# spcl/gemm_hls

Measured on AMD Instinct MI355X. Metric: GFLOP/s, fp32 GEMM N=K=M=16384 per MI355X (tiled outer-product C=A.B), and % of fp32 MFMA peak, higher is better.
Workload: dtype f32; 1 GPU; float 16384x16384x16384 (Multiply,Add) on 1 MI355X; BASELINE configs[1]; kernel=mfma_f32_256x256x16_w8_flush4096, rows_total=16384, rows_per_gpu=16384

## Files before the change

### gemm_hls_amd/csrc/mm_mfma_f32_split.hip

```cpp
#include <mutex>
#include <type_traits>

#include "mm_common.h"

namespace mm {
namespace {

using bf16x8 = __attribute__((ext_vector_type(8))) __bf16;
using f32x4 = __attribute__((ext_vector_type(4))) float;
using f32x16 = __attribute__((ext_vector_type(16))) float;

struct Packed {
  static constexpr int FRAG_BYTES = 64 * 16;
  static constexpr int PLANE_BYTES = 8 * FRAG_BYTES;
  static constexpr int SLAB_BYTES = 3 * PLANE_BYTES;
};
template <int FR_, int WM_, int WN_, int TM_>
struct GeoT {
  static constexpr int FR = FR_, BM = 32 * FR_, BN = 32 * FR_, WM = WM_, WN = WN_, THREADS = 64 * WM_ * WN_;
  static constexpr int TM = TM_, TN = 2, NS = 3;
  static_assert(WM * TM == FR && WN * TN == FR && WM * WN == FR, "one wavefront per fragment and per DMA piece");
  static constexpr int FRAG_BYTES = Packed::FRAG_BYTES;
  static constexpr int PLANE_BYTES = FR * FRAG_BYTES;
  static constexpr int SLAB_BYTES = 3 * PLANE_BYTES;
  static constexpr int STAGE_BYTES = 2 * SLAB_BYTES;
  static constexpr int LDS_BYTES = NS * STAGE_BYTES;
  static constexpr int HALVES = 8 / FR;
};
using GeoS = GeoT<8, 2, 4, 4>;
using GeoS128 = GeoT<4, 2, 2, 2>;

__device__ __forceinline__ void split3(float x, __bf16 &p1, __bf16 &p2, __bf16 &p3) {
  p1 = (__bf16)x;
  const float r1 = x - (float)p1;
  p2 = (__bf16)r1;
  const float r2 = r1 - (float)p2;
  p3 = (__bf16)r2;
  if (!(__builtin_fabsf((float)p1) < __builtin_inff())) {
    p2 = (__bf16)0.0f;
    p3 = (__bf16)0.0f;
  }
}

template <bool ALONG_K, bool PAIRED>
__global__ __launch_bounds__(512) void split_pack_kernel(const float *__restrict__ src, char *__restrict__ dst,
                                                         unsigned rows, unsigned K, unsigned ld, unsigned slabs) {
  const unsigned slab = blockIdx.x, blk = blockIdx.y;
  const unsigned frag = threadIdx.x >> 6, lane = threadIdx.x & 63u;
  const unsigned r = blk * 256 + (PAIRED ? (frag >> 1) * 64 + 2 * (lane & 31u) + (frag & 1u) : frag * 32 + (lane & 31u));
  const unsigned k0 = slab * 16 + (lane >> 5) * 8;
  float x[8];
  if (ALONG_K) {
    if (r < rows && k0 + 8 <= K && (ld & 3u) == 0) {
      const f32x4 lo = *(const f32x4 *)(src + (size_t)r * ld + k0), hi = *(const f32x4 *)(src + (size_t)r * ld + k0 + 4);
#pragma unroll
      for (int e = 0; e < 4; ++e) { x[e] = lo[e]; x[4 + e] = hi[e]; }
    } else {
#pragma unroll
      for (int e = 0; e < 8; ++e) x[e] = (r < rows && k0 + e < K) ? src[(size_t)r * ld + k0 + e] : 0.0f;
    }
  } else {
#pragma unroll
    for (int e = 0; e < 8; ++e) x[e] = (r < rows && k0 + e < K) ? src[(size_t)(k0 + e) * ld + r] : 0.0f;
  }
  bf16x8 p1, p2, p3;
#pragma unroll
  for (int e = 0; e < 8; ++e) {
    __bf16 a, b, c;
    split3(x[e], a, b, c);
    p1[e] = a; p2[e] = b; p3[e] = c;
  }
  char *out = dst + ((size_t)blk * slabs + slab) * Packed::SLAB_BYTES + frag * Packed::FRAG_BYTES + lane * 16;
  *(bf16x8 *)(out) = p1;
  *(bf16x8 *)(out + Packed::PLANE_BYTES) = p2;
  *(bf16x8 *)(out + 2 * Packed::PLANE_BYTES) = p3;
}

__device__ __forceinline__ const char *uniform(const char *p) {
  const unsigned long long v = (unsigned long long)p;
  const unsigned lo = __builtin_amdgcn_readfirstlane((unsigned)v), hi = __builtin_amdgcn_readfirstlane((unsigned)(v >> 32));
  return (const char *)(((unsigned long long)hi << 32) | lo);
}

template <int VAR, int TERMS, class G = GeoS>
__global__ __launch_bounds__(G::THREADS, 2)
void mfma_f32_split_kernel(const char *__restrict__ Ap, const char *__restrict__ Bp, float *__restrict__ C, unsigned N,
                           unsigned M, unsigned slabs, unsigned tiles_n, unsigned tiles_m, unsigned kBand) {
  constexpr int TM = G::TM, TN = G::TN;
  constexpr int NP = TERMS == 6 ? 3 : 2;
  extern __shared__ __attribute__((aligned(16))) char smem[];
  const unsigned lane = threadIdx.x & 63u;
  const unsigned wave = __builtin_amdgcn_readfirstlane(threadIdx.x >> 6);
  constexpr bool PP = (VAR & 64) != 0;
  static_assert(!PP || G::THREADS == 512, "the ping-pong schedule pairs wavefronts w and w+4 of one workgroup");
  const unsigned group = wave >> 2;
  const unsigned wm = PP ? (wave & 3u) >> 1 : wave / G::WN;
  const unsigned wn = PP ? (wave & 1u) * 2 + group : wave % G::WN;
  const unsigned lo = lane & 31u, hi = lane >> 5;

  const unsigned lin = xcd_remap(blockIdx.x, tiles_n * tiles_m);
  const unsigned band = lin / (kBand * tiles_m), within = lin % (kBand * tiles_m);
  const unsigned rows_in_band = min(kBand, tiles_n - band * kBand);
  const unsigned tile_r = band * kBand + within % rows_in_band, tile_c = within / rows_in_band;

  const unsigned voff0 = wave * 1024 + lane * 16, voff1 = voff0 + 8 * 1024, voff2 = voff0 + 16 * 1024;
  const char *a_base = Ap + (size_t)(tile_r / G::HALVES) * slabs * Packed::SLAB_BYTES + (tile_r % G::HALVES) * G::FR * Packed::FRAG_BYTES;
  const char *b_base = Bp + (size_t)(tile_c / G::HALVES) * slabs * Packed::SLAB_BYTES + (tile_c % G::HALVES) * G::FR * Packed::FRAG_BYTES;
  const unsigned lds0 = (unsigned)(size_t)(__attribute__((address_space(3))) char *)smem;
  auto issue = [&](unsigned slab, unsigned buf) {
    const unsigned sl = min(slab, slabs - 1);
    const char *ap = uniform(a_base + (size_t)sl * Packed::SLAB_BYTES), *bp = uniform(b_base + (size_t)sl * Packed::SLAB_BYTES);
    const unsigned la = lds0 + buf * G::STAGE_BYTES + wave * 1024, lb = la + G::SLAB_BYTES;
    unsigned keep;
#define MM_PIECE(vo, sb, la) "s_mov_b32 m0, " la "\n\ts_nop 0\n\tglobal_load_lds_dwordx4 " vo ", " sb "\n\t"
    if constexpr (NP == 3) {
      const unsigned la1 = la + G::PLANE_BYTES, la2 = la + 2 * G::PLANE_BYTES, lb1 = lb + G::PLANE_BYTES, lb2 = lb + 2 * G::PLANE_BYTES;
      asm volatile("s_mov_b32 %0, m0\n\t" MM_PIECE("%1", "%4", "%6") MM_PIECE("%2", "%4", "%7") MM_PIECE("%3", "%4", "%8")
                       MM_PIECE("%1", "%5", "%9") MM_PIECE("%2", "%5", "%10") MM_PIECE("%3", "%5", "%11") "s_mov_b32 m0, %0"
                   : "=&s"(keep)
                   : "v"(voff0), "v"(voff1), "v"(voff2), "s"(ap), "s"(bp), "s"(la), "s"(la1), "s"(la2), "s"(lb), "s"(lb1),
                     "s"(lb2)
                   : "memory");
    } else {
      const unsigned la1 = la + G::PLANE_BYTES, lb1 = lb + G::PLANE_BYTES;
      asm volatile("s_mov_b32 %0, m0\n\t" MM_PIECE("%1", "%3", "%5") MM_PIECE("%2", "%3", "%6") MM_PIECE("%1", "%4", "%7")
                       MM_PIECE("%2", "%4", "%8") "s_mov_b32 m0, %0"
                   : "=&s"(keep)
                   : "v"(voff0), "v"(voff1), "s"(ap), "s"(bp), "s"(la), "s"(la1), "s"(lb), "s"(lb1)
                   : "memory");
    }
#undef MM_PIECE
  };
  constexpr int PIECES = 2 * NP;

  const unsigned a_off = (wm * TM) * G::FRAG_BYTES + lane * 16;
  const unsigned b_off = G::SLAB_BYTES + (wn * TN) * G::FRAG_BYTES + lane * 16;

  f32x16 acc[TM][TN];
#pragma unroll
  for (int mi = 0; mi < TM; ++mi)
#pragma unroll
    for (int ni = 0; ni < TN; ++ni) acc[mi][ni] = (f32x16)0.0f;

  bf16x8 af[2][3], bf[2][TN][3];
  auto read_a = [&](const char *stage, int mi, bf16x8 (&dst)[3]) {
#pragma unroll
    for (int p = 0; p < NP; ++p) dst[p] = *(const bf16x8 *)(stage + a_off + mi * G::FRAG_BYTES + p * G::PLANE_BYTES);
  };
  auto read_b = [&](const char *stage, bf16x8 (&dst)[TN][3]) {
#pragma unroll
    for (int ni = 0; ni < TN; ++ni)
#pragma unroll
      for (int p = 0; p < NP; ++p) dst[ni][p] = *(const bf16x8 *)(stage + b_off + ni * G::FRAG_BYTES + p * G::PLANE_BYTES);
  };
  auto mac = [&](int mi, const bf16x8 (&a)[3], const bf16x8 (&b)[TN][3]) {
    constexpr int PA6[6] = {0, 2, 1, 0, 1, 0}, PB6[6] = {2, 0, 1, 1, 0, 0};
    constexpr int PA3[3] = {0, 1, 0}, PB3[3] = {1, 0, 0};
    if ((VAR & 1) && !(VAR & 16)) __builtin_amdgcn_s_setprio(1);
#pragma unroll
    for (int t = 0; t < TERMS; ++t)
#pragma unroll
      for (int ni = 0; ni < TN; ++ni) {
        const int pa = TERMS == 6 ? PA6[t] : PA3[t % 3], pb = TERMS == 6 ? PB6[t] : PB3[t % 3];
        acc[mi][ni] = __builtin_amdgcn_mfma_f32_32x32x16_bf16(a[pa], b[ni][pb], acc[mi][ni], 0, 0, 0);
      }
    if ((VAR & 1) && !(VAR & 16)) __builtin_amdgcn_s_setprio(0);
  };
  auto sync = [&]() {
    __builtin_amdgcn_sched_barrier(0);
    __builtin_amdgcn_s_barrier();
    __builtin_amdgcn_sched_barrier(0);
  };

  auto stage = [&](auto bufc, auto parc, unsigned s) {
    constexpr int BUF = decltype(bufc)::value, PAR = decltype(parc)::value;
    const char *cur = smem + BUF * G::STAGE_BYTES, *nxt = smem + ((BUF + 1) % 3) * G::STAGE_BYTES;
#pragma unroll
    for (int mi = 0; mi + 1 < TM; ++mi) {
      read_a(cur, mi + 1, af[(mi + 1) & 1]);
      mac(mi, af[mi & 1], bf[PAR]);
    }
    if constexpr (VAR & 16) {
#pragma unroll
      for (int grp = 0; grp + 1 < TM; ++grp) {
#pragma unroll
        for (int i = 0; i < NP; ++i) {
          __builtin_amdgcn_sched_group_barrier(0x008, 1, 0);
          __builtin_amdgcn_sched_group_barrier(0x100, 1, 0);
        }
        __builtin_amdgcn_sched_group_barrier(0x008, 2 * TERMS - NP, 0);
      }
    }
    if constexpr (PIECES == 6) asm volatile("s_waitcnt vmcnt(6)\n\ts_waitcnt lgkmcnt(0)" ::: "memory");
    else asm volatile("s_waitcnt vmcnt(4)\n\ts_waitcnt lgkmcnt(0)" ::: "memory");
    sync();
    issue(s + 3, BUF);
    read_b(nxt, bf[PAR ^ 1]);
    read_a(nxt, 0, af[0]);
    mac(TM - 1, af[(TM - 1) & 1], bf[PAR]);
    if constexpr (VAR & 16) {
      constexpr int READS = (TN + 1) * NP, MFMAS = 2 * TERMS;
#pragma unroll
      for (int i = 0; i < (READS < MFMAS ? READS : MFMAS); ++i) {
        __builtin_amdgcn_sched_group_barrier(0x008, 1, 0);
        __builtin_amdgcn_sched_group_barrier(0x100, 1, 0);
      }
      if (MFMAS > READS) __builtin_amdgcn_sched_group_barrier(0x008, MFMAS - READS, 0);
      else if (READS > MFMAS) __builtin_amdgcn_sched_group_barrier(0x100, READS - MFMAS, 0);
    }
  };

  bf16x8 paf[TM][3];
  auto pp_stage = [&](auto bufc, unsigned s) {
    constexpr int BUF = decltype(bufc)::value;
    const char *cur = smem + BUF * G::STAGE_BYTES;
    read_b(cur, bf[0]);
#pragma unroll
    for (int mi = 0; mi < TM; ++mi) read_a(cur, mi, paf[mi]);
    issue(s + 2, (BUF + 2) % 3);
    if constexpr (PIECES == 6) asm volatile("s_waitcnt vmcnt(6)\n\ts_waitcnt lgkmcnt(0)" ::: "memory");
    else asm volatile("s_waitcnt vmcnt(4)\n\ts_waitcnt lgkmcnt(0)" ::: "memory");
    sync();
    __builtin_amdgcn_s_setprio(1);
#pragma unroll
    for (int mi = 0; mi < TM; ++mi) mac(mi, paf[mi], bf[0]);
    __builtin_amdgcn_s_setprio(0);
    sync();
  };

  const bool shifted = PP && group == 1;
  issue(0, 0);
  issue(1, 1);
  if constexpr (PP) {
    if constexpr (PIECES == 6) asm volatile("s_waitcnt vmcnt(6)" ::: "memory");
    else asm volatile("s_waitcnt vmcnt(4)" ::: "memory");
    sync();
    if (shifted) sync();
  } else {
    issue(2, 2);
    if constexpr (PIECES == 6) asm volatile("s_waitcnt vmcnt(12)" ::: "memory");
    else asm volatile("s_waitcnt vmcnt(8)" ::: "memory");
    sync();
    read_b(smem, bf[0]);
    read_a(smem, 0, af[0]);
  }
  using I0 = std::integral_constant<int, 0>;
  using I1 = std::integral_constant<int, 1>;
  using I2 = std::integral_constant<int, 2>;

  const unsigned row_w = tile_r * G::BM + wm * (TM * 32), col_w = tile_c * G::BN + wn * 64, col = col_w + 2 * lo;
  char *const c_wave = (char *)uniform((const char *)(C + (size_t)row_w * M + col_w));
  const bool pairs = (M & 1u) == 0 && ((size_t)C & 7u) == 0;
  auto writeback = [&](bool accumulate, auto finalc) {
    constexpr bool FINAL = decltype(finalc)::value;
    constexpr int BATCH = FINAL ? 16 : 8;
    using f32x2 = __attribute__((ext_vector_type(2))) float;
    unsigned Mv = M;
    asm volatile("" : "+s"(Mv));
    const unsigned lane_off = (4 * hi * Mv + 2 * lo) * 4u;
    const unsigned rows_left = N > row_w ? N - row_w : 0u;
    const bool interior = pairs && row_w + TM * 32 <= N && col_w + 64 <= M;
    if (interior) {
      typedef __attribute__((address_space(1))) f32x2 *gpair_t;
#pragma unroll
      for (int mi = 0; mi < TM; ++mi)
#pragma unroll
        for (int half = 0; half < 16 / BATCH; ++half) {
          f32x2 old[BATCH];
          if (accumulate) {
#pragma unroll
            for (int j = 0; j < BATCH; ++j) {
              const int rr = half * BATCH + j, lrow = mi * 32 + (rr & 3) + 8 * (rr >> 2);
              old[j] = *(gpair_t)(c_wave + (lane_off + (unsigned)lrow * Mv * 4u));
            }
          } else {
#pragma unroll
            for (int j = 0; j < BATCH; ++j) old[j] = f32x2{0.0f, 0.0f};
          }
#pragma unroll
          for (int j = 0; j < BATCH; ++j) {
            const int rr = half * BATCH + j, lrow = mi * 32 + (rr & 3) + 8 * (rr >> 2);
            *(gpair_t)(c_wave + (lane_off + (unsigned)lrow * Mv * 4u)) = f32x2{acc[mi][0][rr], acc[mi][1][rr]} + old[j];
          }
          if (!FINAL) __builtin_amdgcn_sched_barrier(0);
        }
      return;
    }
#pragma unroll
    for (int mi = 0; mi < TM; ++mi)
#pragma unroll
      for (int half = 0; half < 16 / BATCH; ++half) {
        f32x2 old[BATCH];
#pragma unroll
        for (int j = 0; j < BATCH; ++j) {
          const int rr = half * BATCH + j, lrow = mi * 32 + (rr & 3) + 8 * (rr >> 2);
          const float *src = (const float *)(c_wave + (lane_off + (unsigned)lrow * Mv * 4u));
          const bool row_ok = lrow + 4 * hi < rows_left;
          old[j] = f32x2{0.0f, 0.0f};
          if (accumulate && row_ok) {
            if (pairs) { if (col < M) old[j] = *(const f32x2 *)src; }
            else {
              if (col < M) old[j][0] = src[0];
              if (col + 1 < M) old[j][1] = src[1];
            }
          }
        }
#pragma unroll
        for (int j = 0; j < BATCH; ++j) {
          const int rr = half * BATCH + j, lrow = mi * 32 + (rr & 3) + 8 * (rr >> 2);
          float *dst = (float *)(c_wave + (lane_off + (unsigned)lrow * Mv * 4u));
          const bool row_ok = lrow + 4 * hi < rows_left;
          const f32x2 v = f32x2{acc[mi][0][rr], acc[mi][1][rr]} + old[j];
          if (row_ok) {
            if (pairs) { if (col < M) *(f32x2 *)dst = v; }
            else {
              if (col < M) dst[0] = v[0];
              if (col + 1 < M) dst[1] = v[1];
            }
          }
        }
        if (!FINAL) __builtin_amdgcn_sched_barrier(0);
      }
  };

  constexpr unsigned FC = (VAR & 2) ? ~0u / 2 / 6 * 6 : ((VAR & 32) ? 258 : 516);
  bool flushed = false;
  unsigned c0 = 0, cend = min(FC, slabs);
  for (;;) {
    for (unsigned s = c0; s < cend; s += 6) {
      if constexpr (PP) {
        pp_stage(I0{}, s);
        if (s + 1 < cend) pp_stage(I1{}, s + 1);
        if (s + 2 < cend) pp_stage(I2{}, s + 2);
        if (s + 3 < cend) pp_stage(I0{}, s + 3);
        if (s + 4 < cend) pp_stage(I1{}, s + 4);
        if (s + 5 < cend) pp_stage(I2{}, s + 5);
        continue;
      }
      stage(I0{}, I0{}, s);
      if (s + 1 < cend) stage(I1{}, I1{}, s + 1);
      if (s + 2 < cend) stage(I2{}, I0{}, s + 2);
      if (s + 3 < cend) stage(I0{}, I1{}, s + 3);
      if (s + 4 < cend) stage(I1{}, I0{}, s + 4);
      if (s + 5 < cend) stage(I2{}, I1{}, s + 5);
    }
    if (cend >= slabs) break;
    asm volatile("s_waitcnt vmcnt(0)" ::: "memory");
    writeback(flushed, std::false_type{});
#pragma unroll
    for (int mi = 0; mi < TM; ++mi)
#pragma unroll
      for (int ni = 0; ni < TN; ++ni) acc[mi][ni] = (f32x16)0.0f;
    asm volatile("s_waitcnt vmcnt(0)" ::: "memory");
    flushed = true;
    c0 = cend;
    cend = min(cend + FC, slabs);
  }
  asm volatile("s_waitcnt vmcnt(0)" ::: "memory");
  if (PP && !shifted) sync();
  writeback(flushed, std::true_type{});
}

template <int VAR, int TERMS, class G = GeoS>
int launch_gemm(hipStream_t s, const char *ap, const char *bp, const Problem &p, unsigned slabs) {
  static unsigned long long configured = 0;
  const unsigned tiles_n = (p.n + G::BM - 1) / G::BM, tiles_m = (p.m + G::BN - 1) / G::BN;
  if (int e = ensure_dynamic_lds((const void *)mfma_f32_split_kernel<VAR, TERMS, G>, G::LDS_BYTES, configured)) return e;
  hipLaunchKernelGGL((mfma_f32_split_kernel<VAR, TERMS, G>), dim3(tiles_n * tiles_m), dim3(G::THREADS), G::LDS_BYTES, s, ap,
                     bp, (float *)p.c, p.n, p.m, slabs, tiles_n, tiles_m, band_rows());
  return (int)hipGetLastError();
}

}

bool mfma_f32_split_serves(const Problem &p) { return p.n > 0 && p.m > 0 && p.k > 0 && 132ull * p.m * 4ull < (1ull << 32); }

int mfma_f32_split_tile(const Problem &p, int variant) {
  if (variant > 0 && (variant & 256)) return 256;
  if (variant > 0 && (variant & 512)) return 128;
  static const TileCandidate cands[] = {{256, 256, 256, 1, 1.0}, {128, 128, 128, 2, 0.85}};
  return pick_tile(cands, 2, p.n, p.m);
}

size_t mfma_f32_split_workspace_bytes(const Problem &p) {
  const size_t slabs = (p.k + 15) / 16;
  return ((size_t)((p.n + 255) / 256) + (size_t)((p.m + 255) / 256)) * slabs * Packed::SLAB_BYTES;
}


int launch_mfma_f32_split(hipStream_t s, const Problem &p, int variant) {
  const unsigned slabs = (p.k + 15) / 16;
  const unsigned blocks_a = (p.n + 255) / 256, blocks_b = (p.m + 255) / 256;
  const size_t a_bytes = (size_t)blocks_a * slabs * Packed::SLAB_BYTES, b_bytes = (size_t)blocks_b * slabs * Packed::SLAB_BYTES;
  int dev = 0;
  hipError_t e = hipGetDevice(&dev);
  if (e != hipSuccess) return (int)e;
  hipMemPool_t pool = nullptr;
  if (int rc = workspace_pool(dev, &pool)) return rc;
  char *ws = nullptr;
  const int v = variant < 0 ? 0 : variant;
  if (v & 48) return kErrNotSupported;
  const bool sync_alloc = v & 8;
  if (sync_alloc) e = hipMalloc((void **)&ws, a_bytes + b_bytes);
  else e = hipMallocFromPoolAsync((void **)&ws, a_bytes + b_bytes, pool, s);
  if (e != hipSuccess) return (int)e;
  const float *a = (const float *)p.a, *b = (const float *)p.b;
  (void)hipGetLastError();
  if (p.a_transposed)
    hipLaunchKernelGGL((split_pack_kernel<false, false>), dim3(slabs, blocks_a), dim3(512), 0, s, a, ws, p.n, p.k, p.n, slabs);
  else
    hipLaunchKernelGGL((split_pack_kernel<true, false>), dim3(slabs, blocks_a), dim3(512), 0, s, a, ws, p.n, p.k, p.k, slabs);
  int rc = (int)hipGetLastError();
  if (rc == 0) {
    hipLaunchKernelGGL((split_pack_kernel<false, true>), dim3(slabs, blocks_b), dim3(512), 0, s, b, ws + a_bytes, p.m, p.k, p.m,
                       slabs);
    rc = (int)hipGetLastError();
  }
  if (rc == 0) {
    const char *bp = ws + a_bytes;
    if (v & 1) rc = launch_gemm<1, 6>(s, ws, bp, p, slabs);
    else if ((v & 128) && (v & 4)) rc = launch_gemm<16 | 2, 6>(s, ws, bp, p, slabs);
    else if (v & 128) rc = launch_gemm<16, 6>(s, ws, bp, p, slabs);
    else if (v & 2) rc = launch_gemm<64, 3>(s, ws, bp, p, slabs);
    else if (v & 4) rc = launch_gemm<64 | 2, 6>(s, ws, bp, p, slabs);
    else if (v & 64) rc = launch_gemm<64 | 32, 6>(s, ws, bp, p, slabs);
    else if (mfma_f32_split_tile(p, v) == 128) rc = launch_gemm<16, 6, GeoS128>(s, ws, bp, p, slabs);
    else rc = launch_gemm<64, 6>(s, ws, bp, p, slabs);
  }
  hipError_t f;
  if (sync_alloc) { f = hipStreamSynchronize(s); (void)hipFree(ws); }
  else f = hipFreeAsync(ws, s);
  return rc ? rc : (int)f;
}

}
```

Measured before the change: 150,500 GFLOP/s.

## Switch split-bf16 GEMM body to 16x16x32 MFMA with paired split products

```diff
diff --git a/gemm_hls_amd/csrc/mm_mfma_f32_split.hip b/gemm_hls_amd/csrc/mm_mfma_f32_split.hip
--- a/gemm_hls_amd/csrc/mm_mfma_f32_split.hip
+++ b/gemm_hls_amd/csrc/mm_mfma_f32_split.hip
@@ -42,13 +42,17 @@
   }
 }
 
-template <bool ALONG_K, bool PAIRED>
+template <bool ALONG_K, bool PAIRED, bool H16>
 __global__ __launch_bounds__(512) void split_pack_kernel(const float *__restrict__ src, char *__restrict__ dst,
                                                          unsigned rows, unsigned K, unsigned ld, unsigned slabs) {
   const unsigned slab = blockIdx.x, blk = blockIdx.y;
   const unsigned frag = threadIdx.x >> 6, lane = threadIdx.x & 63u;
-  const unsigned r = blk * 256 + (PAIRED ? (frag >> 1) * 64 + 2 * (lane & 31u) + (frag & 1u) : frag * 32 + (lane & 31u));
-  const unsigned k0 = slab * 16 + (lane >> 5) * 8;
+  const unsigned slot = H16 ? (lane & 15u) + 16 * (lane >> 5) : lane & 31u, kgroup = H16 ? (lane >> 4) & 1u : lane >> 5;
+  const unsigned in_block = !PAIRED ? frag * 32 + slot
+                            : H16   ? frag * 32 + 2 * (slot & 15u) + (slot >> 4)
+                                    : (frag >> 1) * 64 + 2 * slot + (frag & 1u);
+  const unsigned r = blk * 256 + in_block;
+  const unsigned k0 = slab * 16 + kgroup * 8;
   float x[8];
   if (ALONG_K) {
     if (r < rows && k0 + 8 <= K && (ld & 3u) == 0) {
@@ -87,6 +91,8 @@
 void mfma_f32_split_kernel(const char *__restrict__ Ap, const char *__restrict__ Bp, float *__restrict__ C, unsigned N,
                            unsigned M, unsigned slabs, unsigned tiles_n, unsigned tiles_m, unsigned kBand) {
   constexpr int TM = G::TM, TN = G::TN;
+  constexpr bool I32 = (VAR & 128) != 0, SWAP = (VAR & 256) != 0, ADDR = !I32 && !SWAP;
+  static_assert(I32 ? !SWAP : TERMS == 6, "the 16x16x32 body pairs the six products; three products stay on 32x32x16");
   constexpr int NP = TERMS == 6 ? 3 : 2;
   extern __shared__ __attribute__((aligned(16))) char smem[];
   const unsigned lane = threadIdx.x & 63u;
@@ -133,37 +139,86 @@
   };
   constexpr int PIECES = 2 * NP;
 
-  const unsigned a_off = (wm * TM) * G::FRAG_BYTES + lane * 16;
-  const unsigned b_off = G::SLAB_BYTES + (wn * TN) * G::FRAG_BYTES + lane * 16;
-
-  f32x16 acc[TM][TN];
-#pragma unroll
-  for (int mi = 0; mi < TM; ++mi)
-#pragma unroll
-    for (int ni = 0; ni < TN; ++ni) acc[mi][ni] = (f32x16)0.0f;
-
-  bf16x8 af[2][3], bf[2][TN][3];
-  auto read_a = [&](const char *stage, int mi, bf16x8 (&dst)[3]) {
-#pragma unroll
-    for (int p = 0; p < NP; ++p) dst[p] = *(const bf16x8 *)(stage + a_off + mi * G::FRAG_BYTES + p * G::PLANE_BYTES);
-  };
-  auto read_b = [&](const char *stage, bf16x8 (&dst)[TN][3]) {
-#pragma unroll
-    for (int ni = 0; ni < TN; ++ni)
-#pragma unroll
-      for (int p = 0; p < NP; ++p) dst[ni][p] = *(const bf16x8 *)(stage + b_off + ni * G::FRAG_BYTES + p * G::PLANE_BYTES);
-  };
-  auto mac = [&](int mi, const bf16x8 (&a)[3], const bf16x8 (&b)[TN][3]) {
-    constexpr int PA6[6] = {0, 2, 1, 0, 1, 0}, PB6[6] = {2, 0, 1, 1, 0, 0};
-    constexpr int PA3[3] = {0, 1, 0}, PB3[3] = {1, 0, 0};
+  const unsigned a_off = (wm * TM) * G::FRAG_BYTES + (ADDR ? lo : lane) * 16;
+  const unsigned b_off = G::SLAB_BYTES + (wn * TN) * G::FRAG_BYTES + (ADDR ? lo : lane) * 16;
+
+  f32x16 acc32[I32 ? TM : 1][I32 ? TN : 1];
+  f32x4 acc16[I32 ? 1 : 2 * TM][I32 ? 1 : 2 * TN];
+  auto clear = [&]() {
+    if constexpr (I32) {
+#pragma unroll
+      for (int mi = 0; mi < TM; ++mi)
+#pragma unroll
+        for (int ni = 0; ni < TN; ++ni) acc32[mi][ni] = (f32x16)0.0f;
+    } else {
+#pragma unroll
+      for (int mb = 0; mb < 2 * TM; ++mb)
+#pragma unroll
+        for (int nb = 0; nb < 2 * TN; ++nb) acc16[mb][nb] = (f32x4)0.0f;
+    }
+  };
+  clear();
+
+  using u32x4 = __attribute__((ext_vector_type(4))) unsigned;
+  const unsigned sel12 = hi * G::PLANE_BYTES, sel31 = (hi ^ 1u) * 2 * G::PLANE_BYTES;
+  auto read_frag = [&](const char *frag, bf16x8 (&dst)[4]) {
+    if constexpr (I32) {
+#pragma unroll
+      for (int p = 0; p < NP; ++p) dst[p] = *(const bf16x8 *)(frag + p * G::PLANE_BYTES);
+    } else if constexpr (ADDR) {
+      dst[0] = *(const bf16x8 *)(frag + sel12);
+      dst[1] = *(const bf16x8 *)(frag + sel12 + G::FRAG_BYTES / 2);
+      dst[2] = *(const bf16x8 *)(frag + sel31);
+      dst[3] = *(const bf16x8 *)(frag + sel31 + G::FRAG_BYTES / 2);
+    } else {
+      u32x4 p[4];
+#pragma unroll
+      for (int q = 0; q < 3; ++q) p[q] = *(const u32x4 *)(frag + q * G::PLANE_BYTES);
+      p[3] = p[0];
+#pragma unroll
+      for (int i = 0; i < 4; ++i) {
+        const auto s12 = __builtin_amdgcn_permlane32_swap(p[0][i], p[1][i], false, false);
+        p[0][i] = s12[0]; p[1][i] = s12[1];
+        const auto s31 = __builtin_amdgcn_permlane32_swap(p[2][i], p[3][i], false, false);
+        p[2][i] = s31[0]; p[3][i] = s31[1];
+      }
+#pragma unroll
+      for (int q = 0; q < 4; ++q) dst[q] = __builtin_bit_cast(bf16x8, p[q]);
+    }
+  };
+  constexpr int FRAG_READS = I32 ? NP : ADDR ? 4 : 3;
+  constexpr int TILE_MFMAS = I32 ? 2 * TERMS : 3 * 4 * TN;
+
+  bf16x8 af[2][4], bf[2][TN][4];
+  auto read_a = [&](const char *stage, int mi, bf16x8 (&dst)[4]) { read_frag(stage + a_off + mi * G::FRAG_BYTES, dst); };
+  auto read_b = [&](const char *stage, bf16x8 (&dst)[TN][4]) {
+#pragma unroll
+    for (int ni = 0; ni < TN; ++ni) read_frag(stage + b_off + ni * G::FRAG_BYTES, dst[ni]);
+  };
+  auto mac = [&](int mi, const bf16x8 (&a)[4], const bf16x8 (&b)[TN][4]) {
     if ((VAR & 1) && !(VAR & 16)) __builtin_amdgcn_s_setprio(1);
-#pragma unroll
-    for (int t = 0; t < TERMS; ++t)
-#pragma unroll
-      for (int ni = 0; ni < TN; ++ni) {
-        const int pa = TERMS == 6 ? PA6[t] : PA3[t % 3], pb = TERMS == 6 ? PB6[t] : PB3[t % 3];
-        acc[mi][ni] = __builtin_amdgcn_mfma_f32_32x32x16_bf16(a[pa], b[ni][pb], acc[mi][ni], 0, 0, 0);
-      }
+    if constexpr (I32) {
+      constexpr int PA6[6] = {0, 2, 1, 0, 1, 0}, PB6[6] = {2, 0, 1, 1, 0, 0};
+      constexpr int PA3[3] = {0, 1, 0}, PB3[3] = {1, 0, 0};
+#pragma unroll
+      for (int t = 0; t < TERMS; ++t)
+#pragma unroll
+        for (int ni = 0; ni < TN; ++ni) {
+          const int pa = TERMS == 6 ? PA6[t] : PA3[t % 3], pb = TERMS == 6 ? PB6[t] : PB3[t % 3];
+          acc32[mi][ni] = __builtin_amdgcn_mfma_f32_32x32x16_bf16(a[pa], b[ni][pb], acc32[mi][ni], 0, 0, 0);
+        }
+    } else {
+      constexpr int OA[3] = {0, 2, 0}, OB[3] = {2, 0, 0};
+#pragma unroll
+      for (int t = 0; t < 3; ++t)
+#pragma unroll
+        for (int ni = 0; ni < TN; ++ni)
+#pragma unroll
+          for (int h = 0; h < 4; ++h) {
+            f32x4 &c = acc16[2 * mi + (h >> 1)][2 * ni + (h & 1)];
+            c = __builtin_amdgcn_mfma_f32_16x16x32_bf16(a[OA[t] + (h >> 1)], b[ni][OB[t] + (h & 1)], c, 0, 0, 0);
+          }
+    }
     if ((VAR & 1) && !(VAR & 16)) __builtin_amdgcn_s_setprio(0);
   };
   auto sync = [&]() {
@@ -184,11 +239,11 @@
 #pragma unroll
       for (int grp = 0; grp + 1 < TM; ++grp) {
 #pragma unroll
-        for (int i = 0; i < NP; ++i) {
+        for (int i = 0; i < FRAG_READS; ++i) {
           __builtin_amdgcn_sched_group_barrier(0x008, 1, 0);
           __builtin_amdgcn_sched_group_barrier(0x100, 1, 0);
         }
-        __builtin_amdgcn_sched_group_barrier(0x008, 2 * TERMS - NP, 0);
+        __builtin_amdgcn_sched_group_barrier(0x008, TILE_MFMAS - FRAG_READS, 0);
       }
     }
     if constexpr (PIECES == 6) asm volatile("s_waitcnt vmcnt(6)\n\ts_waitcnt lgkmcnt(0)" ::: "memory");
@@ -199,7 +254,7 @@
     read_a(nxt, 0, af[0]);
     mac(TM - 1, af[(TM - 1) & 1], bf[PAR]);
     if constexpr (VAR & 16) {
-      constexpr int READS = (TN + 1) * NP, MFMAS = 2 * TERMS;
+      constexpr int READS = (TN + 1) * FRAG_READS, MFMAS = TILE_MFMAS;
 #pragma unroll
       for (int i = 0; i < (READS < MFMAS ? READS : MFMAS); ++i) {
         __builtin_amdgcn_sched_group_barrier(0x008, 1, 0);
@@ -210,7 +265,7 @@
     }
   };
 
-  bf16x8 paf[TM][3];
+  bf16x8 paf[TM][4];
   auto pp_stage = [&](auto bufc, unsigned s) {
     constexpr int BUF = decltype(bufc)::value;
     const char *cur = smem + BUF * G::STAGE_BYTES;
@@ -248,16 +303,23 @@
   using I1 = std::integral_constant<int, 1>;
   using I2 = std::integral_constant<int, 2>;
 
-  const unsigned row_w = tile_r * G::BM + wm * (TM * 32), col_w = tile_c * G::BN + wn * 64, col = col_w + 2 * lo;
+  const unsigned lane_row = I32 ? 4 * hi : 4 * (lane >> 4), lane_col = I32 ? 2 * lo : 2 * (lane & 15u);
+  const unsigned row_w = tile_r * G::BM + wm * (TM * 32), col_w = tile_c * G::BN + wn * 64, col = col_w + lane_col;
   char *const c_wave = (char *)uniform((const char *)(C + (size_t)row_w * M + col_w));
   const bool pairs = (M & 1u) == 0 && ((size_t)C & 7u) == 0;
+  using f32x2 = __attribute__((ext_vector_type(2))) float;
+  auto item_row = [](int mi, int rr) { return I32 ? mi * 32 + (rr & 3) + 8 * (rr >> 2) : mi * 32 + 16 * (rr >> 3) + (rr & 3); };
+  auto item_col = [](int rr) { return I32 ? 0 : 32 * ((rr >> 2) & 1); };
+  auto item = [&](int mi, int rr) {
+    if constexpr (I32) return f32x2{acc32[mi][0][rr], acc32[mi][1][rr]};
+    else return f32x2{acc16[2 * mi + (rr >> 3)][(rr >> 2) & 1 ? 2 : 0][rr & 3], acc16[2 * mi + (rr >> 3)][(rr >> 2) & 1 ? 3 : 1][rr & 3]};
+  };
   auto writeback = [&](bool accumulate, auto finalc) {
     constexpr bool FINAL = decltype(finalc)::value;
     constexpr int BATCH = FINAL ? 16 : 8;
-    using f32x2 = __attribute__((ext_vector_type(2))) float;
     unsigned Mv = M;
     asm volatile("" : "+s"(Mv));
-    const unsigned lane_off = (4 * hi * Mv + 2 * lo) * 4u;
+    const unsigned lane_off = (lane_row * Mv + lane_col) * 4u;
     const unsigned rows_left = N > row_w ? N - row_w : 0u;
     const bool interior = pairs && row_w + TM * 32 <= N && col_w + 64 <= M;
     if (interior) {
@@ -270,8 +332,8 @@
           if (accumulate) {
 #pragma unroll
             for (int j = 0; j < BATCH; ++j) {
-              const int rr = half * BATCH + j, lrow = mi * 32 + (rr & 3) + 8 * (rr >> 2);
-              old[j] = *(gpair_t)(c_wave + (lane_off + (unsigned)lrow * Mv * 4u));
+              const int rr = half * BATCH + j;
+              old[j] = *(gpair_t)(c_wave + (lane_off + (unsigned)item_row(mi, rr) * Mv * 4u + item_col(rr) * 4u));
             }
           } else {
 #pragma unroll
@@ -279,8 +341,8 @@
           }
 #pragma unroll
           for (int j = 0; j < BATCH; ++j) {
-            const int rr = half * BATCH + j, lrow = mi * 32 + (rr & 3) + 8 * (rr >> 2);
-            *(gpair_t)(c_wave + (lane_off + (unsigned)lrow * Mv * 4u)) = f32x2{acc[mi][0][rr], acc[mi][1][rr]} + old[j];
+            const int rr = half * BATCH + j;
+            *(gpair_t)(c_wave + (lane_off + (unsigned)item_row(mi, rr) * Mv * 4u + item_col(rr) * 4u)) = item(mi, rr) + old[j];
           }
           if (!FINAL) __builtin_amdgcn_sched_barrier(0);
         }
@@ -293,29 +355,31 @@
         f32x2 old[BATCH];
 #pragma unroll
         for (int j = 0; j < BATCH; ++j) {
-          const int rr = half * BATCH + j, lrow = mi * 32 + (rr & 3) + 8 * (rr >> 2);
-          const float *src = (const float *)(c_wave + (lane_off + (unsigned)lrow * Mv * 4u));
-          const bool row_ok = lrow + 4 * hi < rows_left;
+          const int rr = half * BATCH + j, lrow = item_row(mi, rr);
+          const unsigned c = col + item_col(rr);
+          const float *src = (const float *)(c_wave + (lane_off + (unsigned)lrow * Mv * 4u + item_col(rr) * 4u));
+          const bool row_ok = lrow + lane_row < rows_left;
           old[j] = f32x2{0.0f, 0.0f};
           if (accumulate && row_ok) {
-            if (pairs) { if (col < M) old[j] = *(const f32x2 *)src; }
+            if (pairs) { if (c < M) old[j] = *(const f32x2 *)src; }
             else {
-              if (col < M) old[j][0] = src[0];
-              if (col + 1 < M) old[j][1] = src[1];
+              if (c < M) old[j][0] = src[0];
+              if (c + 1 < M) old[j][1] = src[1];
             }
           }
         }
 #pragma unroll
         for (int j = 0; j < BATCH; ++j) {
-          const int rr = half * BATCH + j, lrow = mi * 32 + (rr & 3) + 8 * (rr >> 2);
-          float *dst = (float *)(c_wave + (lane_off + (unsigned)lrow * Mv * 4u));
-          const bool row_ok = lrow + 4 * hi < rows_left;
-          const f32x2 v = f32x2{acc[mi][0][rr], acc[mi][1][rr]} + old[j];
+          const int rr = half * BATCH + j, lrow = item_row(mi, rr);
+          const unsigned c = col + item_col(rr);
+          float *dst = (float *)(c_wave + (lane_off + (unsigned)lrow * Mv * 4u + item_col(rr) * 4u));
+          const bool row_ok = lrow + lane_row < rows_left;
+          const f32x2 v = item(mi, rr) + old[j];
           if (row_ok) {
-            if (pairs) { if (col < M) *(f32x2 *)dst = v; }
+            if (pairs) { if (c < M) *(f32x2 *)dst = v; }
             else {
-              if (col < M) dst[0] = v[0];
-              if (col + 1 < M) dst[1] = v[1];
+              if (c < M) dst[0] = v[0];
+              if (c + 1 < M) dst[1] = v[1];
             }
           }
         }
@@ -347,10 +411,7 @@
     if (cend >= slabs) break;
     asm volatile("s_waitcnt vmcnt(0)" ::: "memory");
     writeback(flushed, std::false_type{});
-#pragma unroll
-    for (int mi = 0; mi < TM; ++mi)
-#pragma unroll
-      for (int ni = 0; ni < TN; ++ni) acc[mi][ni] = (f32x16)0.0f;
+    clear();
     asm volatile("s_waitcnt vmcnt(0)" ::: "memory");
     flushed = true;
     c0 = cend;
@@ -369,6 +430,19 @@
   hipLaunchKernelGGL((mfma_f32_split_kernel<VAR, TERMS, G>), dim3(tiles_n * tiles_m), dim3(G::THREADS), G::LDS_BYTES, s, ap,
                      bp, (float *)p.c, p.n, p.m, slabs, tiles_n, tiles_m, band_rows());
   return (int)hipGetLastError();
+}
+
+template <int FORM>
+int launch_form(hipStream_t s, const char *ap, const char *bp, const Problem &p, unsigned slabs, int v) {
+  if (v & 1) return launch_gemm<FORM | 1, 6>(s, ap, bp, p, slabs);
+  if ((v & 128) && (v & 4)) return launch_gemm<FORM | 16 | 2, 6>(s, ap, bp, p, slabs);
+  if (v & 128) return launch_gemm<FORM | 16, 6>(s, ap, bp, p, slabs);
+  if constexpr (FORM == 128)
+    if (v & 2) return launch_gemm<FORM | 64, 3>(s, ap, bp, p, slabs);
+  if (v & 4) return launch_gemm<FORM | 64 | 2, 6>(s, ap, bp, p, slabs);
+  if (v & 64) return launch_gemm<FORM | 64 | 32, 6>(s, ap, bp, p, slabs);
+  if (mfma_f32_split_tile(p, v) == 128) return launch_gemm<FORM | 16, 6, GeoS128>(s, ap, bp, p, slabs);
+  return launch_gemm<FORM | 64, 6>(s, ap, bp, p, slabs);
 }
 
 }
@@ -406,26 +480,20 @@
   if (e != hipSuccess) return (int)e;
   const float *a = (const float *)p.a, *b = (const float *)p.b;
   (void)hipGetLastError();
-  if (p.a_transposed)
-    hipLaunchKernelGGL((split_pack_kernel<false, false>), dim3(slabs, blocks_a), dim3(512), 0, s, a, ws, p.n, p.k, p.n, slabs);
-  else
-    hipLaunchKernelGGL((split_pack_kernel<true, false>), dim3(slabs, blocks_a), dim3(512), 0, s, a, ws, p.n, p.k, p.k, slabs);
-  int rc = (int)hipGetLastError();
-  if (rc == 0) {
-    hipLaunchKernelGGL((split_pack_kernel<false, true>), dim3(slabs, blocks_b), dim3(512), 0, s, b, ws + a_bytes, p.m, p.k, p.m,
-                       slabs);
-    rc = (int)hipGetLastError();
-  }
+  const bool i32 = (v & 1024) || (v & 2);
+  auto pack = [&](auto along_k, auto paired, const float *src, char *dst, unsigned blocks, unsigned rows, unsigned ld) {
+    constexpr bool AK = decltype(along_k)::value, PR = decltype(paired)::value;
+    if (i32) hipLaunchKernelGGL((split_pack_kernel<AK, PR, false>), dim3(slabs, blocks), dim3(512), 0, s, src, dst, rows, p.k, ld, slabs);
+    else hipLaunchKernelGGL((split_pack_kernel<AK, PR, true>), dim3(slabs, blocks), dim3(512), 0, s, src, dst, rows, p.k, ld, slabs);
+    return (int)hipGetLastError();
+  };
+  int rc = p.a_transposed ? pack(std::false_type{}, std::false_type{}, a, ws, blocks_a, p.n, p.n)
+                          : pack(std::true_type{}, std::false_type{}, a, ws, blocks_a, p.n, p.k);
+  if (rc == 0) rc = pack(std::false_type{}, std::true_type{}, b, ws + a_bytes, blocks_b, p.m, p.m);
   if (rc == 0) {
     const char *bp = ws + a_bytes;
-    if (v & 1) rc = launch_gemm<1, 6>(s, ws, bp, p, slabs);
-    else if ((v & 128) && (v & 4)) rc = launch_gemm<16 | 2, 6>(s, ws, bp, p, slabs);
-    else if (v & 128) rc = launch_gemm<16, 6>(s, ws, bp, p, slabs);
-    else if (v & 2) rc = launch_gemm<64, 3>(s, ws, bp, p, slabs);
-    else if (v & 4) rc = launch_gemm<64 | 2, 6>(s, ws, bp, p, slabs);
-    else if (v & 64) rc = launch_gemm<64 | 32, 6>(s, ws, bp, p, slabs);
-    else if (mfma_f32_split_tile(p, v) == 128) rc = launch_gemm<16, 6, GeoS128>(s, ws, bp, p, slabs);
-    else rc = launch_gemm<64, 6>(s, ws, bp, p, slabs);
+    rc = i32 ? launch_form<128>(s, ws, bp, p, slabs, v) : (v & 2048) ? launch_form<256>(s, ws, bp, p, slabs, v)
+                                                                     : launch_form<0>(s, ws, bp, p, slabs, v);
   }
   hipError_t f;
   if (sync_alloc) { f = hipStreamSynchronize(s); (void)hipFree(ws); }
```

New measurement: 150,500 GFLOP/s, median of 3. No clear change (-0.0%).
